# terraytherapeutics/COATI

Measured on AMD Instinct MI355X. Metric: molecules/sec (contrastive+AR train step), grande_closed, higher is better.
Workload: dtype bf16; 1 GPU; grande_closed d=256 L=16 nh=16 + E3GNN h=256x5, V=10322, batch 1024/GPU, seq_len 80, 16-atom point clouds, InfoNCE + AR loss, bf16 MFMA operands / fp32 accumulate + fp32 master weights, random-init weights; global_batch=1024, seq_len=80, parallelism=dp1

## Files before the change

coati_amd/csrc/engine.cpp:

```cpp
#include <stdarg.h>
#include <stdio.h>
#include <stdlib.h>
#include <string.h>

#include <algorithm>
#include <string>
#include <vector>

#include "../../include/coati_hip.h"
#include "../../include/coati_beam.h"
#include "kernels.h"

#define HIPCHK(x) do { hipError_t _h = (x); if (_h != hipSuccess) { coati_set_error("%s: %s", #x, hipGetErrorString(_h)); return COATI_EHIP; } } while (0)

static thread_local char g_err[512] = "";
void coati_set_error(const char* fmt, ...) {
  va_list ap;
  va_start(ap, fmt);
  vsnprintf(g_err, sizeof(g_err), fmt, ap);
  va_end(ap);
}
extern "C" const char* coati_last_error(void) { return g_err; }
extern "C" int coati_abi_version(void) { return COATI_ABI_VERSION; }

// ... 132 lines not shown
  WgradTile* d_wtab = nullptr;
  int wtab_cap = 0;
  struct WTabKey { const void* pass = nullptr; int lo = -1, hi = -1, M = 0, n = 0; long long sig = 0; };
  WTabKey wtab_key[4];
  const void* wtab_ws = nullptr;
  long long carve_sig = -1;
  int cap_B = 0, cap_T1 = 0, cap_T2 = 0, cap_A = 0;
  WgradTile* h_tab[6] = {nullptr, nullptr, nullptr, nullptr, nullptr, nullptr};
  size_t h_tab_cap[6] = {0, 0, 0, 0, 0, 0};
  hipEvent_t h_tab_ev[6] = {nullptr, nullptr, nullptr, nullptr, nullptr, nullptr};
  int gtab_rr = 0;
  int wtab_rr = 0;
  float* t_dx = nullptr;
  bf16_t *t_dxa = nullptr, *t_dxb = nullptr, *t_dh4 = nullptr, *t_da = nullptr;
  bool gnn_wg_group = false;
  std::vector<bf16_t*> gl_DO16, gl_du, gl_dP;
  WgradTile* d_gtab = nullptr;
  int gtab_cap = 0, gtab_n = 0;
  long long gtab_sig = -1;
  const void* gtab_ws = nullptr;
  float* nce = nullptr;
  size_t nce_cap = 0;
  float* opt_partial;
  float* ln_partial;
  float* ln_part_x;
  ShadowJob* d_jobs = nullptr;
  int* d_tile_start = nullptr;
  std::vector<ShadowJob> jobs;
  std::vector<int> tile_start;
  int n_job_tiles = 0;
  bool jobs_uploaded = false;
  hipStream_t side = nullptr;
  hipEvent_t ev_fork = nullptr, ev_join = nullptr;
  bool gnn_bwd_done = false;
  bool gnn_side_pending = false;
  unsigned long long prof_mask = 0;
  bool prof_paused = false;
  bool prof_keep_overlap = false;
  std::vector<hipEvent_t> ev;
  int ev_used = 0;
  double prof_flops = 0.0;
  double prof_last_bytes = 0.0;
  struct Decode {
    bool active = false;
    int B = 0, Tmax = 0, pos = 0;
    bool ragged = false;
    bf16_t* cache = nullptr;
    float *x = nullptr, *xmid = nullptr, *xn = nullptr, *mean = nullptr, *rstd = nullptr;
    bf16_t *a = nullptr, *qkv = nullptr, *y = nullptr, *hpre = nullptr, *g = nullptr, *af = nullptr;
    int* pos_dev = nullptr;
    long long* tok_dev = nullptr;
    float* inj_dev = nullptr;
    float* logits_dev = nullptr;
    int64_t ldl = 0;
    hipGraphExec_t graph[2] = {nullptr, nullptr};
    int* rope_t = nullptr;
    long long* tok_inj = nullptr;
  } dec;
  double prof_bytes = 0.0;
  double prof_bytes_e = 0.0, prof_flops_e = 0.0;
};

namespace {

bool c2_trains(const coati_engine* e) { return e->enc_to_coati >= 0 && e->G && e->Mo && e->Vo; }
bool c2_refused(const coati_engine* e) { return e->enc_to_coati >= 0 && !c2_trains(e); }
// ... 680 lines not shown
  for (int i = 0; i < 4; ++i)
    if (e->wtab_key[i].pass == &p && e->wtab_key[i].lo == l_lo && e->wtab_key[i].hi == l_hi && e->wtab_key[i].M == Mtab && e->wtab_key[i].sig == sig) slot = i;
  double flops = 0.0, bytes = 0.0;
  for (int l = l_lo; l < l_hi; ++l) {
    flops += 2.0 * M * (3.0 + 1.0 + 4.0 + 4.0) * C * C;
    bytes += (double)M * (3 + 1 + 1 + 1 + 4 + 1 + 1 + 4) * C * 2 + 12.0 * C * C * 8;
  }
  if (slot < 0) {
    std::vector<WgradTile> tab;
    auto add = [&](const bf16_t* A, int lda, const bf16_t* B, int ldb, int N, int K, int64_t w_off, int64_t b_off) -> int {
      WgradArgs a;
      a.A = A; a.lda = lda; a.B = B; a.ldb = ldb; a.M = Mtab; a.N = N; a.K = K; a.dW = e->G + w_off; a.ldw = K; a.dbias = e->G + b_off; a.n_out = 0;
      return wgrad_table_append(tab, a, e->wg_tile);
    };
    for (int l = l_hi - 1; l >= l_lo; --l) {
      const XLayerP& w = e->xl[l];
      COATI_TRY(add(e->w_dqkv[l], 3 * C, p.a1[l], C, 3 * C, C, w.attnw, w.attnb));
      COATI_TRY(add(e->w_dxb[l], C, p.y[l], C, C, C, w.projw, w.projb));
      if (p.tail && l == e->cfg.n_layer_xformer - 1) continue;
      COATI_TRY(add(e->w_dh4[l], 4 * C, p.a2[l], C, 4 * C, C, w.fc1w, w.fc1b));
      COATI_TRY(add(e->w_dxa[l], C, p.g[l], 4 * C, C, 4 * C, w.fc2w, w.fc2b));
    }
    COATI_CHECK_ARG((int)tab.size() <= e->wtab_cap, "wgrad group: table overflow (%zu > %d)", tab.size(), e->wtab_cap);
    slot = e->wtab_rr++ & 3;
    COATI_TRY(upload_table(e, slot, tab, e->d_wtab + (size_t)slot * e->wtab_cap, s, "wgrad group"));
    coati_engine::WTabKey k;
    k.pass = &p; k.lo = l_lo; k.hi = l_hi; k.M = Mtab; k.n = (int)tab.size(); k.sig = sig;
    e->wtab_key[slot] = k;
  }
  ProfScope ps(e, SITE_XF_WGRAD, flops, s, bytes);
  return launch_wgrad_table(e->d_wtab + (size_t)slot * e->wtab_cap, e->wtab_key[slot].n, s, e->wg_tile, M);
}

int xformer_bwd(coati_engine* e, XPass& p, const void* dyf, int dyf_f32, float* dinjection, hipStream_t s, int l_hi = -1, int l_lo = 0,
                const bf16_t* lmh_dlogits = nullptr, bool inputs_only = false) {
  const coati_config& c = e->cfg;
  const int C = c.n_hidden_xformer, L = c.n_layer_xformer, M = p.M;
  if (l_hi < 0) l_hi = L;
  float* DX = e->DX;
  const bool defer = 2 * L + 1 <= COATI_LN_MAX_SLOTS;
  const long long slot_stride = (long long)COATI_LN_PARTIAL_ROWS * 2 * C;
  LnFinishBatch fin;
  memset(&fin, 0, sizeof(fin));
  int nblk = 0;
  auto ln_bwd = [&](const void* dy, int dy_f32, const float* x, const float* mean, const float* rstd, const float* gamma,
                    const float* dres, size_t goff, size_t boff, bf16_t* dx16) -> int {
    if (!defer && inputs_only) return launch_layernorm_bwd(dy, dy_f32, C, x, C, 0, mean, rstd, gamma, dres, DX, dx16, nullptr, nullptr, e->ln_partial, M, C, s);
    if (!defer) return launch_layernorm_bwd(dy, dy_f32, C, x, C, 0, mean, rstd, gamma, dres, DX, dx16, e->G + goff, e->G + boff, e->ln_partial, M, C, s);
    fin.dg_off[fin.n] = (long long)goff;
    fin.db_off[fin.n] = (long long)boff;
    return launch_layernorm_bwd_deferred(dy, dy_f32, C, x, C, 0, mean, rstd, gamma, dres, DX, dx16, e->ln_part_x + (fin.n++) * slot_stride, &nblk, M, C, s);
  };
  auto dgrad_lnbwd = [&](int site, const bf16_t* dY, int K, const bf16_t* WT, const float* x, const float* mean, const float* rstd,
                         const float* gamma, size_t goff, size_t boff, bf16_t* dx16, const bf16_t* chainW = nullptr,
                         bf16_t* chainC = nullptr, bool has_dres = true) -> int {
    if (!defer || c.use_fp8) return 0;
    GemmArgs a;
    memset(&a, 0, sizeof(a));
    a.A = dY; a.lda = K; a.B = WT; a.ldb = K; a.M = M; a.N = C; a.K = K; a.C = DX; a.ldc = C; a.aux_in = has_dres ? DX : nullptr; a.ld_aux = C; a.aux_out = dx16;
    a.lnb_x = x; a.lnb_ldx = C; a.lnb_mean = mean; a.lnb_rstd = rstd; a.lnb_gamma = gamma;
    if (chainW != nullptr && dx16 != nullptr) { a.chain_W = chainW; a.chain_ldw = C; a.chain_C = chainC; a.chain_ldc = C; }
    int nwg = 0;
    if (!lnbwd_rows_supported(a, &nwg) || nwg > COATI_LN_PARTIAL_ROWS) return 0;
    a.lnb_partial = e->ln_part_x + fin.n * slot_stride;
    fin.dg_off[fin.n] = (long long)goff;
    fin.db_off[fin.n] = (long long)boff;
    fin.nblk[fin.n] = nwg;
    ++fin.n;
// ... 69 lines not shown
        ProfScope ps(e, SITE_LN_BWD, 0, s, (double)M * C * (2 + 4 + 4 + 4 + 2));
        COATI_TRY(ln_bwd(e->da, 0, p.xmid[l], p.mean2[l], p.rstd2[l], e->P + w.ln2w, DX, w.ln2w, w.ln2b, dxb));
      }
    }
    if (c.use_fp8) {
      GemmArgs a;
      memset(&a, 0, sizeof(a));
      a.C = e->dyb; a.ldc = C;
      COATI_TRY(gemm8(e, SITE_PROJ_DGRAD, w, 5, dxb, C, M, C, C, a, EPI_BF16, s));
    } else if (!ln2_fused) {
    COATI_TRY(gemm(e, SITE_PROJ_DGRAD, dxb, 0, C, e->S + w.projT, C, M, C, C, e->dyb, C, nullptr, EPI_BF16, nullptr, nullptr, 0, s));
    }
    if (wg_each) COATI_TRY(wgrad(e, SITE_XF_WGRAD, dxb, 0, C, p.y[l], C, M, C, C, e->G + w.projw, C, e->G + w.projb, 0, s));
    {
      ProfScope ps(e, SITE_ATTN_BWD, 10.0 * M * (double)p.T * C, s, (double)M * 8 * C * 2 + (double)M * c.n_head * 8);
      COATI_TRY(launch_attn_bwd(p.qkv[l], p.y[l], e->dyb, p.lse[l], e->attnD, dqkv, e->cos_t, e->sin_t, p.B, p.T, c.n_head, C / c.n_head, s, p.packed ? p.off : nullptr, p.packed ? p.ord : nullptr));
    }
    if (c.use_fp8) {
      GemmArgs a;
      memset(&a, 0, sizeof(a));
      a.C = e->da; a.ldc = C;
      COATI_TRY(gemm8(e, SITE_QKV_DGRAD, w, 4, dqkv, 3 * C, M, C, 3 * C, a, EPI_BF16, s));
    } else {
    ln1_fused = dgrad_lnbwd(SITE_QKV_DGRAD, dqkv, 3 * C, e->S + w.attnT, p.x[l], p.mean1[l], p.rstd1[l], e->P + w.ln1w, w.ln1w, w.ln1b, dx_out);
    if (ln1_fused < 0) return ln1_fused;
    if (!ln1_fused) COATI_TRY(gemm(e, SITE_QKV_DGRAD, dqkv, 0, 3 * C, e->S + w.attnT, 3 * C, M, C, 3 * C, e->da, C, nullptr, EPI_BF16, nullptr, nullptr, 0, s));
    }
    if (wg_each) COATI_TRY(wgrad(e, SITE_XF_WGRAD, dqkv, 0, 3 * C, p.a1[l], C, M, 3 * C, C, e->G + w.attnw, C, e->G + w.attnb, 0, s));
    if (!ln1_fused) {
      ProfScope ps(e, SITE_LN_BWD, 0, s, (double)M * C * (2 + 4 + 4 + 4 + 2));
      COATI_TRY(ln_bwd(e->da, 0, p.x[l], p.mean1[l], p.rstd1[l], e->P + w.ln1w, DX, w.ln1w, w.ln1b, dx_out));
    }
  }
  if (grp && l_hi > l_lo) COATI_TRY(xformer_wgrad_group(e, p, l_lo, l_hi, s));
  if (defer && fin.n > 0 && !inputs_only) {
    ProfScope ps(e, SITE_LN_BWD, 0, s, 0.0);
    COATI_TRY(launch_ln_finish_batched(e->ln_part_x, slot_stride, nblk, e->G, fin, C, s));
  }
  if (l_lo > 0) return COATI_OK;
  ProfScope ps(e, SITE_EMBED, 0, s);
  if (inputs_only) return launch_embed_bwd(p.idx, DX, nullptr, dinjection, c.unk_token, p.B, p.T, C, c.n_tok, s, p.packed ? p.off : nullptr, 1);
  if (c.norm_embed) {
    if (dinjection != nullptr) {
      COATI_TRY(launch_embed_bwd(p.idx, DX, nullptr, dinjection, c.unk_token, p.B, p.T, C, c.n_tok, s, p.packed ? p.off : nullptr, 1));
      COATI_TRY(launch_embed_fwd(p.idx, nullptr, nullptr, c.unk_token, DX, p.B, p.T, C, c.n_tok, s, p.packed ? p.row_src : nullptr, M, 2));
    }
    COATI_TRY(launch_layernorm_bwd(DX, 1, C, p.x_emb, C, 0, p.mean0, p.rstd0, e->P + e->emb_lnw, nullptr, p.x[0], nullptr, e->G + e->emb_lnw, e->G + e->emb_lnb,
                                   e->ln_partial, M, C, s));
    return launch_embed_bwd(p.idx, p.x[0], e->G + e->tok_emb, nullptr, c.unk_token, p.B, p.T, C, c.n_tok, s, p.packed ? p.off : nullptr);
  }
  return launch_embed_bwd(p.idx, DX, e->G + e->tok_emb, dinjection, c.unk_token, p.B, p.T, C, c.n_tok, s, p.packed ? p.off : nullptr);
}

int gnn_fwd(coati_engine* e, const long long* atoms, const float* coords, hipStream_t s) {
  const coati_config& c = e->cfg;
  const int H = c.n_hidden_e3nn, Lg = c.n_layer_e3gnn, B = e->B, A = e->A, BA = B * A, Me = BA * A;
  {
    ProfScope ps(e, SITE_GNN_ELEMWISE, 0, s, (double)BA * (8 + H * 6 + 8) + (double)BA * 12 + (double)Me * 8 * 3 + (double)BA * 4, 20.0);
    bf16_t* h16 = Lg > 0 ? e->g_hcat[0] : e->g_hfin16;
    if (c.torch_emb) COATI_TRY(launch_gnn_embed(atoms, nullptr, nullptr, e->P + e->gembw, nullptr, e->g_h32[0], h16, Lg > 0 ? 2 * H : H, e->g_rstd[0], e->g_mask, BA, H, s, e->err_flag));
    else COATI_TRY(launch_gnn_embed(atoms, e->lut_ix, e->lut_iy, e->P + e->gembw, e->P + e->gembb, e->g_h32[0], h16, Lg > 0 ? 2 * H : H, e->g_rstd[0], e->g_mask, BA, H, s));
    COATI_TRY(launch_gnn_geom(coords, e->g_mask, c.msg_cutoff, e->g_d2, e->g_w, B, A, s));
    COATI_TRY(launch_gnn_compact(e->g_w, e->g_d2, e->g_seg, e->g_ne, e->g_ebj, e->g_ebk, e->g_erev, e->g_ed2, e->g_ew, e->g_pos, B, A, s));
  }
  for (int l = 0; l < Lg; ++l) {
    const GLayerP& w = e->gl[l];
    COATI_TRY(gemm(e, SITE_GNN_NODE_GEMM, e->g_hcat[l], 0, 2 * H, e->S + w.w1ab, H, BA, 2 * H, H, e->g_P[l], 2 * H, nullptr, EPI_BF16, nullptr, nullptr, 0, s));
    if (H == 256) {
      ProfScope ps(e, SITE_GNN_EDGE_GEMM, 0, s, (double)BA * (H * 2 + 4 + H * 2) + (double)H * H * 2, (double)H * 2 + 12 + (double)H * 4, 2.0 * H * H + 6.0 * H);
      COATI_TRY(launch_gnn_edge_fwd_fused(e->g_P[l], 2 * H, e->g_seg, e->g_ebk, e->g_ed2, e->g_ew, e->P + w.e0w + 2 * H, 2 * H + 1, e->P + w.e0b,
                                          e->S + w.e3w, H, e->P + w.e3b, e->g_e1[l], e->g_s2[l], e->g_hcat[l] + H, 2 * H, BA, H, s));
    } else {
    {
      ProfScope ps(e, SITE_GNN_ELEMWISE, 0, s, (double)BA * (H * 2 + 4), (double)H * 4 + 8, 4.0 * H);
      COATI_TRY(launch_gnn_edge_pre_c(e->g_P[l], 2 * H, e->g_seg, e->g_ebk, e->g_ed2, e->P + w.e0w + 2 * H, 2 * H + 1, e->P + w.e0b, e->g_e1[l], BA, H, s));
    }
    {
      GemmArgs a;
      memset(&a, 0, sizeof(a));
      a.m_dev = e->g_ne;
      a.A = e->g_e1[l]; a.lda = H; a.B = e->S + w.e3w; a.ldb = H; a.M = Me; a.N = H; a.K = H; a.C = e->g_s2[l]; a.ldc = H; a.bias = e->P + w.e3b;
      ProfScope ps(e, SITE_GNN_EDGE_GEMM, 0, s, (double)H * H * 2 + H * 4, (double)H * 4, 2.0 * H * H);
      COATI_TRY(launch_gemm_nt(a, 0, EPI_BF16, s));
    }
// ... 108 lines not shown
      ProfScope ps(e, SITE_GNN_ELEMWISE, 0, s, (double)BA * (H * 4 + 4), (double)H * 4 + 8, 4.0 * H);
      COATI_TRY(launch_gnn_edge_pre_bwd_c(e->g_dpre1, e->g_seg, e->g_erev, e->g_ed2, dP, 2 * H, e->G + w.e0w + 2 * H, 2 * H + 1, e->G + w.e0b, BA, H, s));
    }
    COATI_TRY(gemm(e, SITE_GNN_NODE_GEMM, dP, 0, 2 * H, e->S + w.w1abT, 2 * H, BA, H, 2 * H, DO, H, nullptr, EPI_ACC_F32, nullptr, nullptr, 0, s));
    if (!grp) {
      COATI_TRY(wgrad(e, SITE_GNN_WGRAD, dP, 0, 2 * H, e->g_hcat[l], 2 * H, BA, H, H, e->G + w.e0w, 2 * H + 1, nullptr, 0, s));
      COATI_TRY(wgrad(e, SITE_GNN_WGRAD, dP + H, 0, 2 * H, e->g_hcat[l], 2 * H, BA, H, H, e->G + w.e0w + H, 2 * H + 1, nullptr, 0, s));
    }
    float* t = DH; DH = DO; DO = t;
  }
  if (grp) COATI_TRY(gnn_wgrad_group(e, s));
  {
    ProfScope ps(e, SITE_GNN_ELEMWISE, 0, s, (double)BA * (H * 4 + H * 4 + 4 + H * 4) + (double)BA * (8 + H * 4) + 30.0 * H * 4);
    COATI_TRY(launch_layernorm_bwd(DH, 1, H, e->g_h32[0], H, 1, nullptr, e->g_rstd[0], nullptr, nullptr, DO, nullptr, nullptr, nullptr, e->ln_partial, BA, H, s));
    if (e->cfg.torch_emb) COATI_TRY(launch_gnn_embed_bwd(e->atoms, nullptr, nullptr, DO, e->G + e->gembw, nullptr, BA, H, s));
    else COATI_TRY(launch_gnn_embed_bwd(e->atoms, e->lut_ix, e->lut_iy, DO, e->G + e->gembw, e->G + e->gembb, BA, H, s));
  }
  return COATI_OK;
}

int head_linear_bwd(coati_engine* e, SgemmBatch& sb, const float* dY, const float* X, int64_t w_off, int64_t b_off, float* dX, int B,
                    int N, int K) {
  const float* W = e->P + w_off;
  COATI_TRY(sgemm_batch_add(sb, dY, 1, N, X, K, 1, e->G + w_off, K, N, K, B, nullptr, 1.f, 1));
  COATI_TRY(sgemm_batch_add(sb, e->ones, 0, 1, dY, N, 1, e->G + b_off, N, 1, N, B, nullptr, 1.f, 1));
  if (dX) COATI_TRY(sgemm_batch_add(sb, dY, N, 1, W, K, 1, dX, K, B, K, N, nullptr, 1.f, 0));
  return COATI_OK;
}

int ensure_side(coati_engine* e) {
  if (e->side) return COATI_OK;
  if (hipStreamCreateWithFlags(&e->side, hipStreamNonBlocking) != hipSuccess ||
      hipEventCreateWithFlags(&e->ev_fork, hipEventDisableTiming) != hipSuccess ||
      hipEventCreateWithFlags(&e->ev_join, hipEventDisableTiming) != hipSuccess) {
    coati_set_error("engine: could not create the side stream");
    return COATI_EHIP;
  }
  return COATI_OK;
}
int fork_side(coati_engine* e, hipStream_t main) {
  COATI_TRY(ensure_side(e));
  if (hipEventRecord(e->ev_fork, main) != hipSuccess || hipStreamWaitEvent(e->side, e->ev_fork, 0) != hipSuccess) {
    coati_set_error("engine: fork failed");
    return COATI_EHIP;
  }
  return COATI_OK;
}
int join_side(coati_engine* e, hipStream_t main) {
  if (hipEventRecord(e->ev_join, e->side) != hipSuccess || hipStreamWaitEvent(main, e->ev_join, 0) != hipSuccess) {
    coati_set_error("engine: join failed");
    return COATI_EHIP;
  }
  return COATI_OK;
}

int point_head_fwd(coati_engine* e, float* out, hipStream_t s) {
  const coati_config& c = e->cfg;
  const int H = c.n_hidden_e3nn, E = c.n_embd_common, B = e->B;
  if (!c.use_point_encoder) return COATI_OK;
  const float* x = e->hpoint;
  if (c.norm_clips && c.old_architecture) {
    COATI_TRY(launch_sgemm(x, H, 1, e->P + e->p2c_w, 1, H, e->hp_ln, E, B, E, H, e->P + e->p2c_b, 1.f, 0, s));
    return launch_layernorm_fwd(e->hp_ln, E, e->P + e->p2c_lnw, e->P + e->p2c_lnb, nullptr, 0, out, E, e->hp_mean, e->hp_rstd, B, E, s);
  }
  if (c.norm_clips) {
    COATI_TRY(launch_layernorm_fwd(e->hpoint, H, e->P + e->p2c_lnw, e->P + e->p2c_lnb, nullptr, 0, e->hp_ln, H, e->hp_mean, e->hp_rstd, B, H, s));
    x = e->hp_ln;
  }
// ... 142 lines not shown
  COATI_CHECK_ARG(!cfg->use_point_encoder, "engine_create_coati2: COATI2 has no point encoder (use_point_encoder must be 0)");
  COATI_CHECK_ARG(!cfg->use_fp8, "engine_create_coati2: fp8 is not available for COATI2");
  COATI_CHECK_ARG(!cfg->norm_embed, "engine_create_coati2: the COATI2 transformer has no norm_embed");
  const int C = cfg->n_hidden_xformer, E = cfg->n_embd_common;
  COATI_CHECK_SHAPE(E == C, "engine_create_coati2: embed_dim (%d) must equal n_hidden_xformer (%d)", E, C);
  coati_config c = *cfg;
  c.n_layer_e3gnn = 0;
  c.n_hidden_e3nn = C;
  c.norm_clips = 1;
  c.token_mlp = 0;
  c.torch_emb = 0;
  c.old_architecture = 0;
  c.residual = 0;
  COATI_CHECK_SHAPE(c.n_head > 0 && (C == c.n_head * 16 || C == c.n_head * 32), "engine_create_coati2: head size must be 16 or 32 (C=%d, n_head=%d)", C, c.n_head);
  COATI_CHECK_SHAPE(C % 64 == 0 && C <= 1024, "engine_create_coati2: n_hidden_xformer=%d must be a multiple of 64 (<=1024)", C);
  COATI_CHECK_SHAPE(c.n_seq > 0 && c.n_seq <= 256 && c.n_tok > 8, "engine_create_coati2: n_seq must be <= 256");
  COATI_CHECK_SHAPE(c.n_layer_xformer >= 1, "engine_create_coati2: bad layer count");
  coati_engine* e = new coati_engine();
  e->cfg = c;
  e->enc_to_coati = enc_to_coati;
  build_layout(e);
  *out = e;
  return COATI_OK;
}

void coati_engine_destroy(coati_engine* e) {
  if (!e) return;
  for (auto& g : e->dec.graph)
    if (g) hipGraphExecDestroy(g);
  for (auto ev : e->ev) hipEventDestroy(ev);
  if (e->ev_fork) hipEventDestroy(e->ev_fork);
  if (e->ev_join) hipEventDestroy(e->ev_join);
  if (e->side) hipStreamDestroy(e->side);
  for (int i = 0; i < 6; ++i) {
    if (e->h_tab_ev[i]) hipEventDestroy(e->h_tab_ev[i]);
    if (e->h_tab[i]) hipHostFree(e->h_tab[i]);
  }
  delete e;
}

int64_t coati_engine_param_elems(const coati_engine* e) { return e ? e->n_params : 0; }
int64_t coati_engine_trainable_elems(const coati_engine* e) { return e ? e->n_trainable : 0; }
int coati_engine_n_entries(const coati_engine* e) { return e ? (int)e->entries.size() : 0; }
int coati_engine_entry(const coati_engine* e, int i, char* name, int name_cap, int64_t* offset, int32_t* rows, int32_t* cols) {
  COATI_CHECK_ARG(e && i >= 0 && i < (int)e->entries.size() && name && name_cap > 0, "engine_entry: bad argument");
  const Entry& en = e->entries[i];
  snprintf(name, name_cap, "%s", en.name.c_str());
  if (offset) *offset = en.off;
  if (rows) *rows = en.rows;
  if (cols) *cols = en.cols;
  return COATI_OK;
}
int64_t coati_engine_shadow_elems(const coati_engine* e) { return e ? e->n_shadow : 0; }

int coati_engine_reserve(coati_engine* e, int B, int T1, int T2, int A) {
  COATI_CHECK_ARG(e && B >= 0 && T1 >= 0 && T2 >= 0 && A >= 0, "engine_reserve: bad argument");
  COATI_CHECK_SHAPE(T1 <= e->cfg.n_seq && T2 <= e->cfg.n_seq, "engine_reserve: T1=%d T2=%d beyond n_seq=%d", T1, T2, e->cfg.n_seq);
  if (B > e->cap_B) e->cap_B = B;
  if (T1 > e->cap_T1) e->cap_T1 = T1;
  if (T2 > e->cap_T2) e->cap_T2 = T2;
  if (A > e->cap_A) e->cap_A = A;
  return COATI_OK;
}

int64_t coati_engine_workspace_bytes(const coati_engine* e, int B, int T1, int T2, int A, int Bg) {
  if (!e || B <= 0 || T1 <= 0 || T2 <= 0 || A <= 0) return 0;
// ... 433 lines not shown
  float* L2 = L1 + (size_t)B * Bg;
  COATI_TRY(launch_count_valid(bad_all, Bg, scal + 4, scal + 7, s));
  {
    SgemmBatch sb;
    COATI_TRY(sgemm_batch_add(sb, S_loc, E, 1, C_all, 1, E, L1, Bg, B, Bg, E, nullptr, 1.f, 0));
    COATI_TRY(sgemm_batch_add(sb, C_loc, E, 1, S_all, 1, E, L2, Bg, B, Bg, E, nullptr, 1.f, 0));
    COATI_TRY(launch_sgemm_batch(sb, s));
  }
  COATI_TRY(launch_infonce_rows2(L1, L2, Bg, B, Bg, row0, bad_all, scal + 2, scal + 3, scal + 7, gscale, s));
  {
    SgemmBatch sb;
    COATI_TRY(sgemm_batch_add(sb, L1, 1, Bg, S_loc, E, 1, dC_all, E, Bg, E, B, nullptr, 1.f, 0));
    COATI_TRY(sgemm_batch_add(sb, L2, 1, Bg, C_loc, E, 1, dS_all, E, Bg, E, B, nullptr, 1.f, 0));
    COATI_TRY(launch_sgemm_batch(sb, s));
  }
  {
    SgemmBatch sb;
    COATI_TRY(sgemm_batch_add(sb, L1, Bg, 1, C_all, E, 1, dS_all + (size_t)row0 * E, E, B, E, Bg, nullptr, 1.f, 1));
    COATI_TRY(sgemm_batch_add(sb, L2, Bg, 1, S_all, E, 1, dC_all + (size_t)row0 * E, E, B, E, Bg, nullptr, 1.f, 1));
    COATI_TRY(launch_sgemm_batch(sb, s));
  }
  return COATI_OK;
}

int coati_engine_backward(coati_engine* e, const float* dh_smiles, const float* dh_e3gnn, int stage, void* stream) {
  COATI_CHECK_ARG(e && !c2_refused(e), "engine_backward: a COATI2 engine bound without gradient and Adam buffers is inference-only (no backward)");
  COATI_CHECK_ARG(e->have_fwd && e->G, "engine_backward: no forward / gradient buffer");
  COATI_CHECK_ARG(stage >= 0 && stage <= 5, "engine_backward: bad stage");
  const bool c2 = e->enc_to_coati >= 0;
  COATI_CHECK_ARG(!c2 || dh_e3gnn == nullptr, "engine_backward: a COATI2 engine has no point encoder (dh_e3gnn must be null)");
  hipStream_t s = (hipStream_t)stream;
  const coati_config& c = e->cfg;
  const int C = c.n_hidden_xformer, H = c.n_hidden_e3nn, E = c.n_embd_common, B = e->B;
  if (stage == 0 || stage == 1) {
    const int M2 = e->p2.M;
    {
      GemmArgs a;
      memset(&a, 0, sizeof(a));
      a.A = e->p2.af; a.lda = C; a.B = e->S + e->lmhead; a.ldb = C; a.M = M2; a.N = c.n_tok; a.K = C;
      a.C = e->dlogits; a.ldc = e->Vpad; a.n_store = e->Vpad; a.lse = e->ce_lse; a.target = e->p2.packed ? e->p2.ypk : e->y_next; a.scal = e->scal;
      ProfScope ps(e, SITE_LMHEAD_DLOGITS, 2.0 * M2 * c.n_tok * C, s, (double)M2 * C * 2 + (double)c.n_tok * C * 2 + (double)M2 * e->Vpad * 2);
      COATI_TRY(gemm_rows(a, 0, EPI_CE_BWD, s));
    }
    COATI_TRY(wgrad(e, SITE_LMHEAD_WGRAD, e->dlogits, 0, e->Vpad, e->p2.af, C, M2, e->Vpad, C, e->G + e->lmhead, C, nullptr, c.n_tok, s));
    HIPCHK(hipMemsetAsync(e->dcliptok, 0, (size_t)B * E * sizeof(float), s));
    COATI_TRY(xformer_bwd(e, e->p2, e->da, 0, e->dcliptok, s, -1, 0, e->dlogits));
    if (dh_e3gnn) HIPCHK(hipMemcpyAsync(e->dhe, dh_e3gnn, (size_t)B * E * sizeof(float), hipMemcpyDeviceToDevice, s));
    else HIPCHK(hipMemsetAsync(e->dhe, 0, (size_t)B * E * sizeof(float), s));
    if (dh_smiles) HIPCHK(hipMemcpyAsync(e->dhs, dh_smiles, (size_t)B * E * sizeof(float), hipMemcpyDeviceToDevice, s));
    else HIPCHK(hipMemsetAsync(e->dhs, 0, (size_t)B * E * sizeof(float), s));
    if (c2) {
      COATI_TRY(launch_axpy(e->dcliptok, e->dhs, 1.f, (long long)B * E, s));
      COATI_TRY(coati2_head_bwd(e, e->c2t, e->c2t_sv, e->h_smiles, e->dcliptok, e->dhs, e->dhs, B, true, s));
      if (e->enc_to_coati > 0)
        COATI_TRY(coati2_head_bwd(e, e->c2s, e->c2s_sv, e->hstop, e->dhs, e->c2s.residual ? e->dhs : nullptr, e->dhstop, B, true, s));
    } else if (c.token_mlp) {
      HIPCHK(hipMemsetAsync(e->dptok, 0, (size_t)B * E * sizeof(float), s));
      HIPCHK(hipMemsetAsync(e->dstok, 0, (size_t)B * E * sizeof(float), s));
      COATI_TRY(launch_select_rows_bwd(e->use_point, e->dcliptok, e->dptok, e->dstok, B, E, s));
      SgemmBatch sb;
      COATI_TRY(head_linear_bwd(e, sb, e->dptok, e->sa, e->tokw, e->tokb, e->dsa, B, E, E));
      COATI_TRY(head_linear_bwd(e, sb, e->dstok, e->sb, e->tokw, e->tokb, e->dsb, B, E, E));
      COATI_TRY(launch_sgemm_batch(sb, s));
      COATI_TRY(launch_silu_bwd(e->h_e3gnn, e->dsa, e->dhe, (long long)B * E, 1, s));
      COATI_TRY(launch_silu_bwd(e->h_smiles, e->dsb, e->dhs, (long long)B * E, 1, s));
    } else {
      COATI_TRY(launch_select_rows_bwd(e->use_point, e->dcliptok, e->dhe, e->dhs, B, E, s));
    }
    const bool old_arch = c.norm_clips && c.old_architecture;
    if (e->enc_to_coati <= 0) {
    if (old_arch) {
      COATI_TRY(launch_layernorm_bwd(e->dhs, 1, E, e->hs_ln, E, 0, e->hs_mean, e->hs_rstd, e->P + e->s2c_lnw, nullptr, e->dhs_ln, nullptr, e->G + e->s2c_lnw, e->G + e->s2c_lnb, e->ln_partial, B, E, s));
      if (c.use_point_encoder)
        COATI_TRY(launch_layernorm_bwd(e->dhe, 1, E, e->hp_ln, E, 0, e->hp_mean, e->hp_rstd, e->P + e->p2c_lnw, nullptr, e->dhp_ln, nullptr, e->G + e->p2c_lnw, e->G + e->p2c_lnb, e->ln_partial, B, E, s));
    }
    {
      SgemmBatch sb;
      if (old_arch) COATI_TRY(head_linear_bwd(e, sb, e->dhs_ln, e->hstop, e->s2c_w, e->s2c_b, e->dhstop, B, E, C));
      else if (c.norm_clips) COATI_TRY(head_linear_bwd(e, sb, e->dhs, e->hs_ln, e->s2c_w, e->s2c_b, e->dhs_ln, B, E, C));
      else COATI_TRY(head_linear_bwd(e, sb, e->dhs, e->hstop, e->s2c_w, e->s2c_b, e->dhstop, B, E, C));
      if (c.use_point_encoder) {
        if (old_arch) COATI_TRY(head_linear_bwd(e, sb, e->dhp_ln, e->hpoint, e->p2c_w, e->p2c_b, e->dhpoint, B, E, H));
        else if (c.norm_clips) COATI_TRY(head_linear_bwd(e, sb, e->dhe, e->hp_ln, e->p2c_w, e->p2c_b, e->dhp_ln, B, E, H));
        else COATI_TRY(head_linear_bwd(e, sb, e->dhe, e->hpoint, e->p2c_w, e->p2c_b, e->dhpoint, B, E, H));
      }
      COATI_TRY(launch_sgemm_batch(sb, s));
    }
    if (c.norm_clips && !old_arch) {
      COATI_TRY(launch_layernorm_bwd(e->dhs_ln, 1, C, e->hstop, C, 0, e->hs_mean, e->hs_rstd, e->P + e->s2c_lnw, nullptr, e->dhstop, nullptr, e->G + e->s2c_lnw, e->G + e->s2c_lnb, e->ln_partial, B, C, s));
      if (c.use_point_encoder)
        COATI_TRY(launch_layernorm_bwd(e->dhp_ln, 1, H, e->hpoint, H, 0, e->hp_mean, e->hp_rstd, e->P + e->p2c_lnw, nullptr, e->dhpoint, nullptr, e->G + e->p2c_lnw, e->G + e->p2c_lnb, e->ln_partial, B, H, s));
    }
    }
  }
  const int Lx = c.n_layer_xformer, Lmid = Lx / 2;
  const bool ovl_bwd = (stage == 0 || stage == 2 || stage == 4) && (e->prof_mask == 0 || e->prof_keep_overlap) && c.use_point_encoder;
  if (stage == 0 || stage == 1) { e->gnn_bwd_done = false; e->gnn_side_pending = false; }
  if (ovl_bwd) {
    COATI_TRY(fork_side(e, s));
    COATI_TRY(gnn_bwd(e, e->dhpoint, e->side));
  }
  if (stage == 0 || stage == 2 || stage == 4) {
    if (e->p1.tail) {
      COATI_TRY(xformer_bwd(e, e->p1, e->dhstop, 1, nullptr, s, Lx, stage == 4 ? Lmid : 0));
    } else {
      float* dxf = reinterpret_cast<float*>(e->dh4);
      HIPCHK(hipMemsetAsync(dxf, 0, (size_t)e->p1.M * C * sizeof(float), s));
      COATI_TRY(launch_scatter_rows_add(e->dhstop, e->stop_pos, dxf, B, e->T1, C, s, e->p1.packed ? e->p1.off : nullptr));
      COATI_TRY(xformer_bwd(e, e->p1, dxf, 1, nullptr, s, Lx, stage == 4 ? Lmid : 0));
    }
  }
  if (stage == 5) COATI_TRY(xformer_bwd(e, e->p1, nullptr, 1, nullptr, s, Lmid, 0));
  if (ovl_bwd && stage == 4) {
    e->gnn_side_pending = true;
  } else if (ovl_bwd || (stage == 5 && e->gnn_side_pending)) {
    COATI_TRY(join_side(e, s));
    e->gnn_bwd_done = true;
    e->gnn_side_pending = false;
  } else if ((stage == 0 || stage == 3) && !e->gnn_bwd_done) {
    if (c.use_point_encoder) COATI_TRY(gnn_bwd(e, e->dhpoint, s));
    e->gnn_bwd_done = true;
  }
  return COATI_OK;
}

int coati_engine_optimizer_step(coati_engine* e, float lr, float beta1, float beta2, float eps, float weight_decay,
                                float max_norm, int step, float* scal, void* stream) {
  COATI_CHECK_ARG(e && !c2_refused(e), "optimizer_step: a COATI2 engine bound without gradient and Adam buffers is inference-only (no optimizer step)");
  COATI_CHECK_ARG(e->P && e->G && e->Mo && e->Vo && scal, "optimizer_step: engine not bound for training");
  COATI_CHECK_ARG(e->have_fwd, "optimizer_step: needs the workspace of a forward call");
  hipStream_t s = (hipStream_t)stream;
  {
    ProfScope ps(e, SITE_OPTIM, 0, s);
    COATI_TRY(launch_grad_sqnorm(e->G, e->n_trainable, e->opt_partial, 1024, scal + 5, max_norm, scal + 8, s));
    COATI_TRY(launch_adamw(e->P, e->G, e->Mo, e->Vo, e->S, e->n_trainable, lr, beta1, beta2, eps, weight_decay, step, scal + 8, 1.f, s, e->err_flag));
  }
  return refresh_shadows_impl(e, stream, true);
}

int coati_engine_set_error_word(coati_engine* e, const int32_t* word_dev, void* stream) {
  COATI_CHECK_ARG(e && word_dev && e->have_ws && e->err_flag && e->scal, "set_error_word: no forward workspace");
  hipStream_t s = (hipStream_t)stream;
  if (hipMemcpyAsync(e->err_flag, word_dev, sizeof(int), hipMemcpyDeviceToDevice, s) != hipSuccess ||
      hipMemcpyAsync(e->scal + 6, word_dev, sizeof(int), hipMemcpyDeviceToDevice, s) != hipSuccess) {
    coati_set_error("set_error_word: copy failed");
// ... 339 lines not shown
```

Before: 49250 molecules/s.

## Overlap transformer backward tails and contrastive heads with wgrad via side streams

Adds a second non-blocking stream with per-pass fork and join events. After the last dgrad layer of each transformer backward, the layernorm-finish, embedding backward and (for the decoder pass) the contrastive head backward now run on a side stream. Meanwhile the grouped weight-gradient GEMM keeps running on the main stream. The goal is to hide these small latency-bound kernels behind the wgrad work, at the cost of extra event synchronisation and possible races on shared scratch buffers such as ln_partial.

```diff
diff --git a/coati_amd/csrc/engine.cpp b/coati_amd/csrc/engine.cpp
--- a/coati_amd/csrc/engine.cpp
+++ b/coati_amd/csrc/engine.cpp
@@ -188,6 +188,8 @@
   bool jobs_uploaded = false;
   hipStream_t side = nullptr;
   hipEvent_t ev_fork = nullptr, ev_join = nullptr;
+  hipStream_t seam = nullptr;
+  hipEvent_t ev_sfork[2] = {nullptr, nullptr}, ev_sjoin[2] = {nullptr, nullptr};
   bool gnn_bwd_done = false;
   bool gnn_side_pending = false;
   unsigned long long prof_mask = 0;
@@ -934,8 +936,10 @@
   return launch_wgrad_table(e->d_wtab + (size_t)slot * e->wtab_cap, e->wtab_key[slot].n, s, e->wg_tile, M);
 }
 
+int seam_fork(coati_engine* e, int pass, hipStream_t main, hipStream_t to);
 int xformer_bwd(coati_engine* e, XPass& p, const void* dyf, int dyf_f32, float* dinjection, hipStream_t s, int l_hi = -1, int l_lo = 0,
-                const bf16_t* lmh_dlogits = nullptr, bool inputs_only = false) {
+                const bf16_t* lmh_dlogits = nullptr, bool inputs_only = false, hipStream_t seam = nullptr, int seam_pass = 0,
+                bool* seam_forked = nullptr) {
   const coati_config& c = e->cfg;
   const int C = c.n_hidden_xformer, L = c.n_layer_xformer, M = p.M;
   if (l_hi < 0) l_hi = L;
@@ -1071,24 +1075,30 @@
       COATI_TRY(ln_bwd(e->da, 0, p.x[l], p.mean1[l], p.rstd1[l], e->P + w.ln1w, DX, w.ln1w, w.ln1b, dx_out));
     }
   }
+  hipStream_t ts = s;
+  if (grp && l_hi > l_lo && l_lo == 0 && seam != nullptr) {
+    COATI_TRY(seam_fork(e, seam_pass, s, seam));
+    ts = seam;
+    if (seam_forked) *seam_forked = true;
+  }
   if (grp && l_hi > l_lo) COATI_TRY(xformer_wgrad_group(e, p, l_lo, l_hi, s));
   if (defer && fin.n > 0 && !inputs_only) {
-    ProfScope ps(e, SITE_LN_BWD, 0, s, 0.0);
-    COATI_TRY(launch_ln_finish_batched(e->ln_part_x, slot_stride, nblk, e->G, fin, C, s));
+    ProfScope ps(e, SITE_LN_BWD, 0, ts, 0.0);
+    COATI_TRY(launch_ln_finish_batched(e->ln_part_x, slot_stride, nblk, e->G, fin, C, ts));
   }
   if (l_lo > 0) return COATI_OK;
-  ProfScope ps(e, SITE_EMBED, 0, s);
-  if (inputs_only) return launch_embed_bwd(p.idx, DX, nullptr, dinjection, c.unk_token, p.B, p.T, C, c.n_tok, s, p.packed ? p.off : nullptr, 1);
+  ProfScope ps(e, SITE_EMBED, 0, ts);
+  if (inputs_only) return launch_embed_bwd(p.idx, DX, nullptr, dinjection, c.unk_token, p.B, p.T, C, c.n_tok, ts, p.packed ? p.off : nullptr, 1);
   if (c.norm_embed) {
     if (dinjection != nullptr) {
-      COATI_TRY(launch_embed_bwd(p.idx, DX, nullptr, dinjection, c.unk_token, p.B, p.T, C, c.n_tok, s, p.packed ? p.off : nullptr, 1));
-      COATI_TRY(launch_embed_fwd(p.idx, nullptr, nullptr, c.unk_token, DX, p.B, p.T, C, c.n_tok, s, p.packed ? p.row_src : nullptr, M, 2));
+      COATI_TRY(launch_embed_bwd(p.idx, DX, nullptr, dinjection, c.unk_token, p.B, p.T, C, c.n_tok, ts, p.packed ? p.off : nullptr, 1));
+      COATI_TRY(launch_embed_fwd(p.idx, nullptr, nullptr, c.unk_token, DX, p.B, p.T, C, c.n_tok, ts, p.packed ? p.row_src : nullptr, M, 2));
     }
     COATI_TRY(launch_layernorm_bwd(DX, 1, C, p.x_emb, C, 0, p.mean0, p.rstd0, e->P + e->emb_lnw, nullptr, p.x[0], nullptr, e->G + e->emb_lnw, e->G + e->emb_lnb,
-                                   e->ln_partial, M, C, s));
-    return launch_embed_bwd(p.idx, p.x[0], e->G + e->tok_emb, nullptr, c.unk_token, p.B, p.T, C, c.n_tok, s, p.packed ? p.off : nullptr);
-  }
-  return launch_embed_bwd(p.idx, DX, e->G + e->tok_emb, dinjection, c.unk_token, p.B, p.T, C, c.n_tok, s, p.packed ? p.off : nullptr);
+                                   e->ln_partial, M, C, ts));
+    return launch_embed_bwd(p.idx, p.x[0], e->G + e->tok_emb, nullptr, c.unk_token, p.B, p.T, C, c.n_tok, ts, p.packed ? p.off : nullptr);
+  }
+  return launch_embed_bwd(p.idx, DX, e->G + e->tok_emb, dinjection, c.unk_token, p.B, p.T, C, c.n_tok, ts, p.packed ? p.off : nullptr);
 }
 
 int gnn_fwd(coati_engine* e, const long long* atoms, const float* coords, hipStream_t s) {
@@ -1263,8 +1273,27 @@
   if (e->side) return COATI_OK;
   if (hipStreamCreateWithFlags(&e->side, hipStreamNonBlocking) != hipSuccess ||
       hipEventCreateWithFlags(&e->ev_fork, hipEventDisableTiming) != hipSuccess ||
-      hipEventCreateWithFlags(&e->ev_join, hipEventDisableTiming) != hipSuccess) {
-    coati_set_error("engine: could not create the side stream");
+      hipEventCreateWithFlags(&e->ev_join, hipEventDisableTiming) != hipSuccess ||
+      hipStreamCreateWithFlags(&e->seam, hipStreamNonBlocking) != hipSuccess ||
+      hipEventCreateWithFlags(&e->ev_sfork[0], hipEventDisableTiming) != hipSuccess ||
+      hipEventCreateWithFlags(&e->ev_sfork[1], hipEventDisableTiming) != hipSuccess ||
+      hipEventCreateWithFlags(&e->ev_sjoin[0], hipEventDisableTiming) != hipSuccess ||
+      hipEventCreateWithFlags(&e->ev_sjoin[1], hipEventDisableTiming) != hipSuccess) {
+    coati_set_error("engine: could not create the side streams");
+    return COATI_EHIP;
+  }
+  return COATI_OK;
+}
+int seam_fork(coati_engine* e, int pass, hipStream_t main, hipStream_t to) {
+  if (hipEventRecord(e->ev_sfork[pass], main) != hipSuccess || hipStreamWaitEvent(to, e->ev_sfork[pass], 0) != hipSuccess) {
+    coati_set_error("engine: seam fork failed");
+    return COATI_EHIP;
+  }
+  return COATI_OK;
+}
+int seam_join(coati_engine* e, int pass, hipStream_t main, hipStream_t from) {
+  if (hipEventRecord(e->ev_sjoin[pass], from) != hipSuccess || hipStreamWaitEvent(main, e->ev_sjoin[pass], 0) != hipSuccess) {
+    coati_set_error("engine: seam join failed");
     return COATI_EHIP;
   }
   return COATI_OK;
@@ -1473,6 +1502,11 @@
   if (e->ev_fork) hipEventDestroy(e->ev_fork);
   if (e->ev_join) hipEventDestroy(e->ev_join);
   if (e->side) hipStreamDestroy(e->side);
+  for (int i = 0; i < 2; ++i) {
+    if (e->ev_sfork[i]) hipEventDestroy(e->ev_sfork[i]);
+    if (e->ev_sjoin[i]) hipEventDestroy(e->ev_sjoin[i]);
+  }
+  if (e->seam) hipStreamDestroy(e->seam);
   for (int i = 0; i < 6; ++i) {
     if (e->h_tab_ev[i]) hipEventDestroy(e->h_tab_ev[i]);
     if (e->h_tab[i]) hipHostFree(e->h_tab[i]);
@@ -1972,6 +2006,8 @@
   hipStream_t s = (hipStream_t)stream;
   const coati_config& c = e->cfg;
   const int C = c.n_hidden_xformer, H = c.n_hidden_e3nn, E = c.n_embd_common, B = e->B;
+  const bool seam_on = e->prof_mask == 0 || e->prof_keep_overlap;
+  bool heads_on_side = false;
   if (stage == 0 || stage == 1) {
     const int M2 = e->p2.M;
     {
@@ -1984,35 +2020,38 @@
     }
     COATI_TRY(wgrad(e, SITE_LMHEAD_WGRAD, e->dlogits, 0, e->Vpad, e->p2.af, C, M2, e->Vpad, C, e->G + e->lmhead, C, nullptr, c.n_tok, s));
     HIPCHK(hipMemsetAsync(e->dcliptok, 0, (size_t)B * E * sizeof(float), s));
-    COATI_TRY(xformer_bwd(e, e->p2, e->da, 0, e->dcliptok, s, -1, 0, e->dlogits));
-    if (dh_e3gnn) HIPCHK(hipMemcpyAsync(e->dhe, dh_e3gnn, (size_t)B * E * sizeof(float), hipMemcpyDeviceToDevice, s));
-    else HIPCHK(hipMemsetAsync(e->dhe, 0, (size_t)B * E * sizeof(float), s));
-    if (dh_smiles) HIPCHK(hipMemcpyAsync(e->dhs, dh_smiles, (size_t)B * E * sizeof(float), hipMemcpyDeviceToDevice, s));
-    else HIPCHK(hipMemsetAsync(e->dhs, 0, (size_t)B * E * sizeof(float), s));
+    bool seam = false;
+    if (seam_on) COATI_TRY(ensure_side(e));
+    COATI_TRY(xformer_bwd(e, e->p2, e->da, 0, e->dcliptok, s, -1, 0, e->dlogits, false, seam_on ? e->side : nullptr, 0, &seam));
+    const hipStream_t hs = seam ? e->side : s;
+    if (dh_e3gnn) HIPCHK(hipMemcpyAsync(e->dhe, dh_e3gnn, (size_t)B * E * sizeof(float), hipMemcpyDeviceToDevice, hs));
+    else HIPCHK(hipMemsetAsync(e->dhe, 0, (size_t)B * E * sizeof(float), hs));
+    if (dh_smiles) HIPCHK(hipMemcpyAsync(e->dhs, dh_smiles, (size_t)B * E * sizeof(float), hipMemcpyDeviceToDevice, hs));
+    else HIPCHK(hipMemsetAsync(e->dhs, 0, (size_t)B * E * sizeof(float), hs));
     if (c2) {
-      COATI_TRY(launch_axpy(e->dcliptok, e->dhs, 1.f, (long long)B * E, s));
-      COATI_TRY(coati2_head_bwd(e, e->c2t, e->c2t_sv, e->h_smiles, e->dcliptok, e->dhs, e->dhs, B, true, s));
+      COATI_TRY(launch_axpy(e->dcliptok, e->dhs, 1.f, (long long)B * E, hs));
+      COATI_TRY(coati2_head_bwd(e, e->c2t, e->c2t_sv, e->h_smiles, e->dcliptok, e->dhs, e->dhs, B, true, hs));
       if (e->enc_to_coati > 0)
-        COATI_TRY(coati2_head_bwd(e, e->c2s, e->c2s_sv, e->hstop, e->dhs, e->c2s.residual ? e->dhs : nullptr, e->dhstop, B, true, s));
+        COATI_TRY(coati2_head_bwd(e, e->c2s, e->c2s_sv, e->hstop, e->dhs, e->c2s.residual ? e->dhs : nullptr, e->dhstop, B, true, hs));
     } else if (c.token_mlp) {
-      HIPCHK(hipMemsetAsync(e->dptok, 0, (size_t)B * E * sizeof(float), s));
-      HIPCHK(hipMemsetAsync(e->dstok, 0, (size_t)B * E * sizeof(float), s));
-      COATI_TRY(launch_select_rows_bwd(e->use_point, e->dcliptok, e->dptok, e->dstok, B, E, s));
+      HIPCHK(hipMemsetAsync(e->dptok, 0, (size_t)B * E * sizeof(float), hs));
+      HIPCHK(hipMemsetAsync(e->dstok, 0, (size_t)B * E * sizeof(float), hs));
+      COATI_TRY(launch_select_rows_bwd(e->use_point, e->dcliptok, e->dptok, e->dstok, B, E, hs));
       SgemmBatch sb;
       COATI_TRY(head_linear_bwd(e, sb, e->dptok, e->sa, e->tokw, e->tokb, e->dsa, B, E, E));
       COATI_TRY(head_linear_bwd(e, sb, e->dstok, e->sb, e->tokw, e->tokb, e->dsb, B, E, E));
-      COATI_TRY(launch_sgemm_batch(sb, s));
-      COATI_TRY(launch_silu_bwd(e->h_e3gnn, e->dsa, e->dhe, (long long)B * E, 1, s));
-      COATI_TRY(launch_silu_bwd(e->h_smiles, e->dsb, e->dhs, (long long)B * E, 1, s));
+      COATI_TRY(launch_sgemm_batch(sb, hs));
+      COATI_TRY(launch_silu_bwd(e->h_e3gnn, e->dsa, e->dhe, (long long)B * E, 1, hs));
+      COATI_TRY(launch_silu_bwd(e->h_smiles, e->dsb, e->dhs, (long long)B * E, 1, hs));
     } else {
-      COATI_TRY(launch_select_rows_bwd(e->use_point, e->dcliptok, e->dhe, e->dhs, B, E, s));
+      COATI_TRY(launch_select_rows_bwd(e->use_point, e->dcliptok, e->dhe, e->dhs, B, E, hs));
     }
     const bool old_arch = c.norm_clips && c.old_architecture;
     if (e->enc_to_coati <= 0) {
     if (old_arch) {
-      COATI_TRY(launch_layernorm_bwd(e->dhs, 1, E, e->hs_ln, E, 0, e->hs_mean, e->hs_rstd, e->P + e->s2c_lnw, nullptr, e->dhs_ln, nullptr, e->G + e->s2c_lnw, e->G + e->s2c_lnb, e->ln_partial, B, E, s));
+      COATI_TRY(launch_layernorm_bwd(e->dhs, 1, E, e->hs_ln, E, 0, e->hs_mean, e->hs_rstd, e->P + e->s2c_lnw, nullptr, e->dhs_ln, nullptr, e->G + e->s2c_lnw, e->G + e->s2c_lnb, e->ln_partial, B, E, hs));
       if (c.use_point_encoder)
-        COATI_TRY(launch_layernorm_bwd(e->dhe, 1, E, e->hp_ln, E, 0, e->hp_mean, e->hp_rstd, e->P + e->p2c_lnw, nullptr, e->dhp_ln, nullptr, e->G + e->p2c_lnw, e->G + e->p2c_lnb, e->ln_partial, B, E, s));
+        COATI_TRY(launch_layernorm_bwd(e->dhe, 1, E, e->hp_ln, E, 0, e->hp_mean, e->hp_rstd, e->P + e->p2c_lnw, nullptr, e->dhp_ln, nullptr, e->G + e->p2c_lnw, e->G + e->p2c_lnb, e->ln_partial, B, E, hs));
     }
     {
       SgemmBatch sb;
@@ -2024,33 +2063,41 @@
         else if (c.norm_clips) COATI_TRY(head_linear_bwd(e, sb, e->dhe, e->hp_ln, e->p2c_w, e->p2c_b, e->dhp_ln, B, E, H));
         else COATI_TRY(head_linear_bwd(e, sb, e->dhe, e->hpoint, e->p2c_w, e->p2c_b, e->dhpoint, B, E, H));
       }
-      COATI_TRY(launch_sgemm_batch(sb, s));
+      COATI_TRY(launch_sgemm_batch(sb, hs));
     }
     if (c.norm_clips && !old_arch) {
-      COATI_TRY(launch_layernorm_bwd(e->dhs_ln, 1, C, e->hstop, C, 0, e->hs_mean, e->hs_rstd, e->P + e->s2c_lnw, nullptr, e->dhstop, nullptr, e->G + e->s2c_lnw, e->G + e->s2c_lnb, e->ln_partial, B, C, s));
+      COATI_TRY(launch_layernorm_bwd(e->dhs_ln, 1, C, e->hstop, C, 0, e->hs_mean, e->hs_rstd, e->P + e->s2c_lnw, nullptr, e->dhstop, nullptr, e->G + e->s2c_lnw, e->G + e->s2c_lnb, e->ln_partial, B, C, hs));
       if (c.use_point_encoder)
-        COATI_TRY(launch_layernorm_bwd(e->dhp_ln, 1, H, e->hpoint, H, 0, e->hp_mean, e->hp_rstd, e->P + e->p2c_lnw, nullptr, e->dhpoint, nullptr, e->G + e->p2c_lnw, e->G + e->p2c_lnb, e->ln_partial, B, H, s));
-    }
-    }
+        COATI_TRY(launch_layernorm_bwd(e->dhp_ln, 1, H, e->hpoint, H, 0, e->hp_mean, e->hp_rstd, e->P + e->p2c_lnw, nullptr, e->dhpoint, nullptr, e->G + e->p2c_lnw, e->G + e->p2c_lnb, e->ln_partial, B, H, hs));
+    }
+    }
+    if (seam) COATI_TRY(seam_join(e, 0, s, e->side));
+    heads_on_side = seam;
   }
   const int Lx = c.n_layer_xformer, Lmid = Lx / 2;
   const bool ovl_bwd = (stage == 0 || stage == 2 || stage == 4) && (e->prof_mask == 0 || e->prof_keep_overlap) && c.use_point_encoder;
   if (stage == 0 || stage == 1) { e->gnn_bwd_done = false; e->gnn_side_pending = false; }
   if (ovl_bwd) {
-    COATI_TRY(fork_side(e, s));
+    if (!heads_on_side) COATI_TRY(fork_side(e, s));
     COATI_TRY(gnn_bwd(e, e->dhpoint, e->side));
   }
+  auto enc_bwd = [&](const void* dyf, int l_hi, int l_lo) -> int {
+    bool seam = false;
+    if (seam_on) COATI_TRY(ensure_side(e));
+    COATI_TRY(xformer_bwd(e, e->p1, dyf, 1, nullptr, s, l_hi, l_lo, nullptr, false, seam_on ? e->seam : nullptr, 1, &seam));
+    return seam ? seam_join(e, 1, s, e->seam) : COATI_OK;
+  };
   if (stage == 0 || stage == 2 || stage == 4) {
     if (e->p1.tail) {
-      COATI_TRY(xformer_bwd(e, e->p1, e->dhstop, 1, nullptr, s, Lx, stage == 4 ? Lmid : 0));
+      COATI_TRY(enc_bwd(e->dhstop, Lx, stage == 4 ? Lmid : 0));
     } else {
       float* dxf = reinterpret_cast<float*>(e->dh4);
       HIPCHK(hipMemsetAsync(dxf, 0, (size_t)e->p1.M * C * sizeof(float), s));
       COATI_TRY(launch_scatter_rows_add(e->dhstop, e->stop_pos, dxf, B, e->T1, C, s, e->p1.packed ? e->p1.off : nullptr));
-      COATI_TRY(xformer_bwd(e, e->p1, dxf, 1, nullptr, s, Lx, stage == 4 ? Lmid : 0));
-    }
-  }
-  if (stage == 5) COATI_TRY(xformer_bwd(e, e->p1, nullptr, 1, nullptr, s, Lmid, 0));
+      COATI_TRY(enc_bwd(dxf, Lx, stage == 4 ? Lmid : 0));
+    }
+  }
+  if (stage == 5) COATI_TRY(enc_bwd(nullptr, Lmid, 0));
   if (ovl_bwd && stage == 4) {
     e->gnn_side_pending = true;
   } else if (ovl_bwd || (stage == 5 && e->gnn_side_pending)) {
```

Result: no change. 49540 molecules/s, median of 6 (+0.6%).
